# autonomousvision/transfuser

Hardware: AMD Instinct MI355X
Metric: training samples/sec (RGB+LiDAR pair), bs=10/GPU (higher is better)
Workload: dtype f32; 1 GPU; TransFuser LidarCenterNet (RegNetY-3.2GF x2, 168.0 M params) full train step, B=10/GPU, 3x256x704 RGB + 3x256x256 BEV, fp32, dropout 0.10, hipGraph replay; global_batch=10, parallelism=dp1, grad_allreduce=none (1 rank), build_id=e9ad36df01ded5b2

## Files before the change

### include/transfuser_hip.h

```cpp
#ifndef TRANSFUSER_HIP_H
#define TRANSFUSER_HIP_H
#include <stdint.h>
#ifdef __cplusplus
extern "C" {
#endif

int tf_version(void);
const char* tf_last_error(void);
const char* tf_build_id(void);
long tf_streamk_launches(void);

int tf_set_precision(int mode);
int tf_get_precision(void);
int tf_autotune(int enable);
int tf_force_plan(int bm, int bn, int bk, int splitk);
int tf_force_dma(int kind, int splitk);
int tf_plans_count(void);
int tf_plans_clear(void);
int tf_plans_save(const char* path);
int tf_plans_load(const char* path);


typedef struct {
    const float* a; const float* b; float* c; const float* bias; const float* res;
// ... 12 lines not shown
int tf_gemm_f32(const tf_gemm_desc* d, void* stream);
long tf_gemm_splitk_ws_floats(const tf_gemm_desc* d);
int tf_gemm_pair_begin(void);
int tf_gemm_pair_end(void* stream);
long tf_gemm_pair_count(int singles);

typedef struct {
    int B, Hi, Wi, Cin, Ho, Wo, Cout, ksize, stride, pad, groups;
} tf_conv_geom;
int tf_conv2d_fwd_f32(const tf_conv_geom* g, const float* x, const float* w, const float* bias, float* y, int relu, void* stream);
int tf_conv2d_fwd_colstat_f32(const tf_conv_geom* g, const float* x, const float* w, const float* bias, float* y, float* colstat, int* colstat_nparts,
                              void* stream);
int tf_conv2d_dgrad_f32(const tf_conv_geom* g, const float* dy, const float* w, float* dx, int accumulate, void* stream);
int tf_conv2d_wgrad_f32(const tf_conv_geom* g, const float* dy, const float* x, float* dw, int accumulate, void* stream);

int tf_conv3x3_small_fwd_f32(const float* x, const float* w, const float* bias, float* y, int B, int H, int W, int Cin, int Cout, int relu, void* stream);
int tf_conv3x3_small_dgrad_f32(const float* dy, const float* w, float* dx, int B, int H, int W, int Cin, int Cout, int accumulate, void* stream);
long tf_conv3x3_small_wgrad_ws_floats(void);
int tf_conv3x3_small_wgrad_f32(const float* dy, const float* x, float* dw, int B, int H, int W, int Cin, int Cout, int accumulate, float* ws, void* stream);

int tf_bn_finalize_parts_f32(const float* parts, int nparts, int rows, int C, const float* gamma, const float* beta, float* running_mean, float* running_var,
                             float momentum, float eps, float* save_mean, float* save_invstd, float* coef_out, void* stream);
int tf_colsum_bnrelu_parts_f32(const float* x, const float* coef, int nseg, int rows_per_seg, int C, float* ws, int* nchunks, void* stream);
int tf_se_excite_fwd_parts_f32(const float* parts, int nchunks, float scale, const float* W1, const float* b1, const float* W2, const float* b2, int B, int C,
                               int Cr, float* s_out, float* g1, float* gate, float* bwd_scratch, void* stream);
int tf_se_scale_bn_fwd_f32(const float* x, const float* coef, const float* gate, float* y, int B, int HW, int C, void* stream);
int tf_se_gate_grad_parts_f32(const float* dy, const float* x, const float* coef, int B, int HW, int C, float* ws, int* nchunks, void* stream);
int tf_se_excite_bwd_parts_f32(const float* parts, int nchunks, const float* gate, const float* s, const float* g1, const float* W1, const float* W2, int B,
                               int C, int Cr, float* dW1, float* db1, float* dW2, float* db2, float* ds, float* scratch, int scratch_is_zero, void* stream);
int tf_bn_bwd_remask_f32(const float* dz, const float* x, const float* fwd_coef, int rows, int C, const float* gamma, const float* save_mean,
                         const float* save_invstd, float* dx, float* dgamma, float* dbeta, float* ws, void* stream);
int tf_bn_bwd_remask_se_f32(const float* dy, const float* gate, const float* dmean, int B, int HW, int C, const float* x, const float* fcoef, const float* gamma,
                            const float* save_mean, const float* save_invstd, float* dx, float* dgamma, float* dbeta, float* ws, void* stream);

int tf_dwconv7_fwd_f32(const float* x, const float* w, const float* bias, float* y, int B, int H, int W, int C, int flip, int accumulate, void* stream);
int tf_dwconv7_wgrad_f32(const float* dy, const float* x, float* dw, float* dbias, int B, int H, int W, int C, void* stream);
int tf_gelu_fwd_f32(const float* x, float* y, int64_t n, void* stream);
int tf_gelu_bwd_f32(const float* dy, const float* x, float* dx, int64_t n, void* stream);
int tf_colscale_add_f32(const float* x, const float* gamma, const float* beta, const float* res, float* y, int64_t rows, int C, void* stream);
int tf_colsum_mul_f32(const float* a, const float* b, int rows, int C, float* out, int accumulate, float* ws, void* stream);
int tf_colsum_multi_f32(int n, const float* const* xs, const int* Cs, const long* lds, float* const* outs, int rows, void* stream);

int tf_cast16_f32(const float* x, int rows, int cols, int ldx, void* y16, int ldy, void* y16t, int ldyt, int dtype, void* stream);
typedef struct { const float* x; void* y16; void* y16t; int rows, cols, ldx, ldy, ldyt, tile0; } tf_cast16_item;
int tf_cast16_multi_f32(const tf_cast16_item* items_dev, int n_items, int total_tiles, int dtype, void* stream);
int tf_bn_apply16_f32(const float* x, const float* coef, const float* res, int relu, float* y32, int rows, int C, void* y16, void* y16t, int ldyt, int dtype, void* stream);
int tf_se_scale_bn16_f32(const float* x, const float* coef, const float* gate, int B, int HW, int C, void* y16, void* y16t, int ldyt, int dtype, void* stream);
int tf_bn_bwd16_f32(const float* dz, const float* z, const float* x, int rows, int C, const float* gamma, const float* save_mean, const float* save_invstd, float* dx32,
                    float* dres, float* dgamma, float* dbeta, float* ws, void* dx16, void* dx16t, int ldyt, int dtype, void* stream);
int tf_bn_bwd_remask16_f32(const float* dz, const float* x, const float* fcoef, int rows, int C, const float* gamma, const float* save_mean, const float* save_invstd,
                           float* dx32, float* dgamma, float* dbeta, float* ws, void* dx16, void* dx16t, int ldyt, int dtype, void* stream);
int tf_layernorm_fwd16_f32(const float* x, const float* gamma, const float* beta, void* y16, int ldy, void* y16t, int ldyt, float* mean, float* rstd,
                           int rows, int C, float eps, int dtype, void* stream);
int tf_gemm16_nt_f32(const void* a16, const void* b16, float* c, int m, int n, int k, int lda, int ldb, int ldc, const float* bias, const float* res, int ldres,
                     float alpha, int relu, int accumulate, const float* mask, int ldmask, int dtype, void* stream);
int tf_gemm16_nt_colstat_f32(const void* a16, const void* b16, float* c, int m, int n, int k, int lda, int ldb, int ldc, int dtype, float* colstat,
                             int* colstat_nparts, void* stream);
int tf_add_strided2_f32(const float* src, float* dst, int B, int Ho, int Wo, int C, int Hi, int Wi, void* stream);
int tf_im2col3x3_f32(const float* x, float* cols, int B, int H, int W, int C, void* stream);

int tf_conv3x3_thin_supported(int Cin, int Cout);
int tf_conv3x3_thin_fwd_f32(const float* x, const float* w, const float* bias, float* y, int B, int H, int W, int Cin, int Cout, void* stream);
int tf_conv3x3_thin_dgrad_f32(const float* dy, const float* w, const float* relu_mask, float* dx, int B, int H, int W, int Cin, int Cout, int accumulate,
                              void* stream);
long tf_conv3x3_thin_wgrad_ws_floats(void);
int tf_conv3x3_thin_wgrad_f32(const float* dy, const float* x, float* dw, float* dbias, int B, int H, int W, int Cin, int Cout, int accumulate, float* ws,
// ... 171 lines not shown
```

### transfuser_amd/csrc/reduce.cpp

```cpp
#include <cstdlib>
#include "tf_common.h"
#include "../../include/transfuser_hip.h"

using namespace tf;

namespace {

template <int V> struct vecf { float v[V]; };
template <int V> __device__ __forceinline__ vecf<V> ldv(const float* p) {
    vecf<V> r;
    if (V == 4) { float4 t = *reinterpret_cast<const float4*>(p); r.v[0] = t.x; r.v[1 % V] = t.y; r.v[2 % V] = t.z; r.v[3 % V] = t.w; }
    else r.v[0] = *p;
    return r;
}
template <int V> __device__ __forceinline__ void stv(float* p, const vecf<V>& a) {
    if (V == 4) *reinterpret_cast<float4*>(p) = make_float4(a.v[0], a.v[1 % V], a.v[2 % V], a.v[3 % V]);
    else *p = a.v[0];
}

constexpr int kBnSlots = 16;
constexpr int kMaxChunks = 512;
constexpr long kWsFloats = 4L << 20;
constexpr int kTickets = 4096;

// ... 593 lines not shown
    int e = 0;
#pragma unroll
    for (int i = 1; i < kMultiMax; ++i)
        if (i < d.n && (int)blockIdx.x >= d.strip0[i]) e = i;
    const int tx = threadIdx.x & 7, ty = threadIdx.x >> 3;
    const int C = d.C[e];
    const int c = ((int)blockIdx.x - d.strip0[e]) * 32 + tx * 4;
    const bool live = c < C;
    const float* p = d.x[e] + (live ? c : 0);
    const long ld = d.ld[e];
    float4 acc = make_float4(0.f, 0.f, 0.f, 0.f);
    int r = ty;
    for (; r + 7 * 32 < rows; r += 8 * 32) {
        float4 v[8];
#pragma unroll
        for (int u = 0; u < 8; ++u) v[u] = *reinterpret_cast<const float4*>(p + (long)(r + 32 * u) * ld);
#pragma unroll
        for (int u = 0; u < 8; ++u) { acc.x += v[u].x; acc.y += v[u].y; acc.z += v[u].z; acc.w += v[u].w; }
    }
    for (; r < rows; r += 32) {
        const float4 v = *reinterpret_cast<const float4*>(p + (long)r * ld);
        acc.x += v.x; acc.y += v.y; acc.z += v.z; acc.w += v.w;
    }
    red[ty][tx] = acc;
    __syncthreads();
    if (ty == 0 && live) {
        float4 t = make_float4(0.f, 0.f, 0.f, 0.f);
        for (int j = 0; j < 32; ++j) { const float4 v = red[j][tx]; t.x += v.x; t.y += v.y; t.z += v.z; t.w += v.w; }
        float* o = d.out[e] + c;
        o[0] += t.x; o[1] += t.y; o[2] += t.z; o[3] += t.w;
    }
}

constexpr int T16S = 64, T16P = T16S + 8;
template <class F>
__global__ void __launch_bounds__(256) tile16_kernel(F f, int rows, int C, uint16_t* __restrict__ y, uint16_t* __restrict__ yt, long ldyt, int f16) {
    __shared__ __attribute__((aligned(16))) uint16_t T[T16S * T16P];
    const int tid = threadIdx.x, r0 = blockIdx.y * T16S, c0 = blockIdx.x * T16S, c4 = (tid & 15) * 4;
#pragma unroll
    for (int it = 0; it < 4; ++it) {
        const int row = it * 16 + (tid >> 4), r = r0 + row, c = c0 + c4;
        float v[4] = {0.f, 0.f, 0.f, 0.f};
        const bool in = r < rows && c < C;
        if (in) f(r, c, v);
        uint16_t h[4];
#pragma unroll
        for (int e = 0; e < 4; ++e) h[e] = cvt16_bits(v[e], f16 != 0);
        if (y && in) *reinterpret_cast<float2*>(y + (long)r * C + c) = make_float2(__uint_as_float((uint32_t)h[0] | ((uint32_t)h[1] << 16)), __uint_as_float((uint32_t)h[2] | ((uint32_t)h[3] << 16)));
        if (yt) {
#pragma unroll
            for (int e = 0; e < 4; ++e) T[(c4 + e) * T16P + row] = h[e];
        }
    }
    if (!yt) return;
    __syncthreads();
    const int rows8 = (rows + 7) & ~7;
#pragma unroll
    for (int p = 0; p < 2; ++p) {
        const int id = p * 256 + tid, col = id >> 3, rc = (id & 7) * 8;
        if (c0 + col < C && r0 + rc < rows8) *reinterpret_cast<float4*>(yt + (long)(c0 + col) * ldyt + r0 + rc) = *reinterpret_cast<const float4*>(T + col * T16P + rc);
    }
}
struct BnApply16F {
    const float* x; const float* coef; const float* res; float* y32; int C; int relu;
    __device__ __forceinline__ void operator()(int r, int c, float (&v)[4]) const {
        const long o = (long)r * C + c;
// ... 229 lines not shown
    const bool v4 = (C % 4 == 0) && aligned16(dz) && aligned16(x) && aligned16(dx) && aligned16(fcoef);
    RedPlan p = plan_reduce(rows, C, 1, 2, v4);
    BnBwdRemaskF<4> f4{dz, x, fcoef, save_mean, save_invstd, C};
    BnBwdRemaskF<1> f1{dz, x, fcoef, save_mean, save_invstd, C};
    launch_reduce<2>(p, f4, f1, rows, C, 1, ws, stream);
    TF_LAUNCH(bn_bwd_finalize_kernel, dim3(cdiv(C, 4)), dim3(256), stream, (const float*)ws, gamma, save_mean, save_invstd, dgamma, dbeta, coef, C, p.nchunks,
              (float)rows);
    const long n = (long)rows * C;
    if (v4) TF_LAUNCH(bn_bwd_apply_remask_kernel<4>, dim3(ew_blocks(n / 4)), dim3(256), stream, dz, x, fcoef, (const float*)coef, dx, n / 4, C);
    else TF_LAUNCH(bn_bwd_apply_remask_kernel<1>, dim3(ew_blocks(n)), dim3(256), stream, dz, x, fcoef, (const float*)coef, dx, n, C);
    return launch_status("tf_bn_bwd_remask_f32");
}

extern "C" int tf_bn_bwd_remask_se_f32(const float* dy, const float* gate, const float* dmean, int B, int HW, int C, const float* x, const float* fcoef,
                                       const float* gamma, const float* save_mean, const float* save_invstd, float* dx, float* dgamma, float* dbeta, float* ws,
                                       void* stream) {
    TF_REQUIRE(dy && gate && dmean && x && fcoef && gamma && save_mean && save_invstd && dx && ws && B > 0 && HW > 0 && C > 0, "tf_bn_bwd_remask_se_f32: bad arguments");
    const int rows = B * HW;
    float* coef = ws + kWsFloats / 2;
    const bool v4 = (C % 4 == 0) && aligned16(dy) && aligned16(x) && aligned16(dx) && aligned16(fcoef) && aligned16(gate) && aligned16(dmean);
    RedPlan p = plan_reduce(rows, C, 1, 2, v4);
    const float inv_hw = 1.f / (float)HW;
    SeBnBwdRemaskF<4> f4{dy, gate, dmean, x, fcoef, save_mean, save_invstd, C, HW, inv_hw};
    SeBnBwdRemaskF<1> f1{dy, gate, dmean, x, fcoef, save_mean, save_invstd, C, HW, inv_hw};
    launch_reduce<2>(p, f4, f1, rows, C, 1, ws, stream);
    TF_LAUNCH(bn_bwd_finalize_kernel, dim3(cdiv(C, 4)), dim3(256), stream, (const float*)ws, gamma, save_mean, save_invstd, dgamma, dbeta, coef, C, p.nchunks,
              (float)rows);
    const long n = (long)rows * C;
    if (v4) TF_LAUNCH(bn_bwd_apply_remask_se_kernel<4>, dim3(ew_blocks(n / 4)), dim3(256), stream, dy, gate, dmean, x, fcoef, (const float*)coef, dx, n / 4, C, (long)HW * C / 4, inv_hw);
    else TF_LAUNCH(bn_bwd_apply_remask_se_kernel<1>, dim3(ew_blocks(n)), dim3(256), stream, dy, gate, dmean, x, fcoef, (const float*)coef, dx, n, C, (long)HW * C, inv_hw);
    return launch_status("tf_bn_bwd_remask_se_f32");
}

extern "C" int tf_colsum_mul_f32(const float* a, const float* b, int rows, int C, float* out, int accumulate, float* ws, void* stream) {
    TF_REQUIRE(a && b && out && ws && rows > 0 && C > 0, "tf_colsum_mul_f32: bad arguments");
    RedPlan p = plan_reduce(rows, C, 1, 1, aligned16(a) && aligned16(b));
    MulF<4> f4{a, b, C};
    MulF<1> f1{a, b, C};
    launch_reduce<1>(p, f4, f1, rows, C, 1, ws, stream);
    TF_LAUNCH(colsum_finalize_kernel, dim3(cdiv((long)C, 4)), dim3(256), stream, (const float*)ws, out, C, p.nchunks, 1, 1.f, accumulate);
    return launch_status("tf_colsum_mul_f32");
}

extern "C" int tf_colsum_multi_f32(int n, const float* const* xs, const int* Cs, const long* lds, float* const* outs, int rows, void* stream) {
    TF_REQUIRE(n >= 1 && n <= kMultiMax && xs && Cs && lds && outs && rows > 0, "tf_colsum_multi_f32: 1 <= n <= %d matrices with rows > 0", kMultiMax);
    MultiSum d;
    d.n = n;
    int strips = 0;
    for (int i = 0; i < kMultiMax; ++i) {
        const int j = i < n ? i : n - 1;
        d.x[i] = xs[j]; d.out[i] = outs[j]; d.C[i] = Cs[j]; d.ld[i] = lds[j];
        d.strip0[i] = strips;
        if (i < n) {
            TF_REQUIRE(xs[i] && outs[i] && Cs[i] > 0 && Cs[i] % 4 == 0 && lds[i] % 4 == 0 && lds[i] >= Cs[i] && aligned16(xs[i]),
                       "tf_colsum_multi_f32: entry %d needs C %% 4 == 0, ld %% 4 == 0, ld >= C and a 16-byte aligned base", i);
            strips += cdiv(Cs[i], 32);
        }
    }
    d.strip0[kMultiMax] = strips;
    TF_LAUNCH(colsum_multi_kernel, dim3(strips), dim3(256), stream, d, rows);
    return launch_status("tf_colsum_multi_f32");
}

extern "C" int tf_bn_apply16_f32(const float* x, const float* coef, const float* res, int relu, float* y32, int rows, int C, void* y16, void* y16t, int ldyt,
                                 int dtype, void* stream) {
    TF_REQUIRE(x && coef && tile16_ok(rows, C, y16, y16t, ldyt, dtype) && aligned16(x) && aligned16(coef) && (!res || aligned16(res)) && (!y32 || aligned16(y32)),
// ... 44 lines not shown
```

### transfuser_amd/functions.py

```python
import math

import torch

from . import ops


_INPLACE = False
_collect = None


class inplace_param_grads:
    def __enter__(self):
        global _INPLACE
        self.prev, _INPLACE = _INPLACE, True

    def __exit__(self, *a):
        global _INPLACE
        _INPLACE = self.prev


def gbuf(p):
    if _collect is not None:
        t = _collect.get(id(p))
        if t is None:
# ... 27 lines not shown
        finally:
            _collect = prev

    cls.forward, cls.backward = staticmethod(forward), staticmethod(backward)
    return cls


def w2d(w):
    return w.view(w.shape[0], w.shape[1])


def bias_grad(dy2d, b, mask2d=None):
    ops.colsum(dy2d, 1, dy2d.shape[0], dy2d.shape[1], 1.0, mask=mask2d, out=gbuf(b).view(1, -1), accumulate=True)


def _bn(x, bn, res=None, relu=False, stat=None):
    grp = getattr(bn, "_sync_group", None)
    if grp is None and isinstance(bn, torch.nn.SyncBatchNorm) and bn.training:
        import torch.distributed as dist
        if dist.is_available() and dist.is_initialized() and dist.get_world_size(bn.process_group) > 1:
            grp = bn.process_group if bn.process_group is not None else dist.group.WORLD
    if grp is not None and bn.training:
        return _bn_sync_fwd(x, bn, res, relu, grp)
    if stat is not None and bn.training:
        y, sm, si = ops.bn_fwd_parts(x, stat, bn.weight, bn.bias, bn.running_mean, bn.running_var, res, relu, bn.momentum, bn.eps)
        return y, (sm, si)
    y, sm, si = ops.bn_fwd(x, bn.weight, bn.bias, bn.running_mean, bn.running_var, res, relu, bn.training, bn.momentum, bn.eps)
    return y, (sm, si)


def _bn_bwd(dz, z, x, bn, st, want_dres=False):
    if len(st) == 4:
        return _bn_sync_bwd(dz, z, x, bn, st, want_dres)
    return ops.bn_bwd(dz, z, x, bn.weight, st[0], st[1], gbuf(bn.weight), gbuf(bn.bias), want_dres)


def convert_sync_batchnorm(model, group=None):
    import torch.distributed as dist
    grp = group if group is not None else dist.group.WORLD
    for m in model.modules():
        if isinstance(m, torch.nn.modules.batchnorm._BatchNorm):
            m._sync_group = grp
    return model


def _bn_sync_fwd(x, bn, res, relu, grp):
    import torch.distributed as dist
    C = x.shape[-1]
    n = x.numel() // C
    _, m_loc, i_loc = ops.bn_fwd(x, bn.weight, bn.bias, None, None, None, False, True, bn.momentum, bn.eps)
    world = dist.get_world_size(grp)
    mine = torch.cat([m_loc.double(), (1.0 / (i_loc.double() * i_loc.double()) - bn.eps).clamp_(min=0.0), torch.full((1,), float(n), dtype=torch.float64, device=x.device)])
    allst = [torch.empty_like(mine) for _ in range(world)]
    dist.all_gather(allst, mine, group=grp)
    cnt = torch.stack([t[2 * C] for t in allst])
    means = torch.stack([t[:C] for t in allst]); varis = torch.stack([t[C:2 * C] for t in allst])
    N = cnt.sum()
    mean = (means * cnt[:, None]).sum(0) / N
    var = ((varis + (means - mean) ** 2) * cnt[:, None]).sum(0) / N
    mean32, var32 = mean.float(), var.float()
    y, _, _ = ops.bn_fwd(x, bn.weight, bn.bias, mean32, var32, res, relu, False, bn.momentum, bn.eps)
    if bn.running_mean is not None:
        with torch.no_grad():
            mom = bn.momentum
            Nf = float(N)
            bn.running_mean.mul_(1 - mom).add_(mean32, alpha=mom)
            bn.running_var.mul_(1 - mom).add_(var32 * (Nf / (Nf - 1)) if Nf > 1 else var32, alpha=mom)
# ... 299 lines not shown
        else:
            out, st3 = _bn(y3, bn3, res=sc, relu=True, stat=cs3)
        ctx.saved = (x, blk, y1, z1, st1, y2, z2, st2, s, g1, gate, z2ss, y3, st3, yd, std, out, x2s, (lp, x16t, z16t))
        return out

    @staticmethod
    def backward(ctx, dout):
        if ctx.saved is None:
            raise RuntimeError("YBlockFn: trying to backward through the graph a second time: the saved activations are freed by the first backward "
                               "(retain_graph is not supported by the block Functions)")
        x, blk, y1, z1, st1, y2, z2, st2, s, g1, gate, z2ss, y3, st3, yd, std, out, x2s, (lp, x16t, z16t) = ctx.saved
        B, H, W, Cin = x.shape
        _, Ho, Wo, C = out.shape
        x2 = x.view(-1, Cin)
        w3 = blk.conv3.conv.weight
        if lp:
            bn3 = blk.conv3.bn
            if len(st3) == 2:
                _, d16, d16t, dsc = ops.bn_bwd16(dout.contiguous(), out, y3, bn3.weight, st3[0], st3[1], gbuf(bn3.weight), gbuf(bn3.bias), want_dres=True)
            else:
                dy3, dsc = _bn_bwd(dout.contiguous(), out, y3, bn3, st3, want_dres=True)
                d16, d16t = ops.cast16(dy3.view(-1, C))
            dz2s = _c1x1_bwd16(d16, d16t, z16t, w2d(w3), w2d(gbuf(w3))).view(B, Ho, Wo, C)
        else:
            dy3, dsc = _bn_bwd(dout.contiguous(), out, y3, blk.conv3.bn, st3, want_dres=True)
            dy3_2 = dy3.view(-1, C)
            dz2s = _c1x1_bwd(dy3_2, z2ss, w2d(w3), w2d(gbuf(w3))).view(B, Ho, Wo, C)
        se = blk.se
        if z2 is None:
            ds = ops.se_gate_excite_bn_bwd(dz2s, y2, st2[2], gate, s, g1, se.fc1.weight, se.fc2.weight, gbuf(se.fc1.weight), gbuf(se.fc1.bias),
                                           gbuf(se.fc2.weight), gbuf(se.fc2.bias))
            bn2 = blk.conv2.bn
            if ops.FUSE_SE_BN_BWD:
                dy2 = ops.bn_bwd_remask_se(dz2s, gate, ds, y2, st2[2], bn2.weight, st2[0], st2[1], gbuf(bn2.weight), gbuf(bn2.bias))
            else:
                dz2 = ops.se_scale_bwd_x(dz2s, gate, ds, y2.shape)
                dy2 = ops.bn_bwd_remask(dz2, y2, st2[2], bn2.weight, st2[0], st2[1], gbuf(bn2.weight), gbuf(bn2.bias))
        else:
            dgate = ops.se_scale_bwd_gate(dz2s, z2, gate)
            if B <= 16 and C <= ops.SE_FUSED_MAX_C and B * g1.shape[1] <= 8192:
                ds = ops.se_excite_bwd(dgate, s, g1, se.fc1.weight, se.fc2.weight, gbuf(se.fc1.weight), gbuf(se.fc1.bias), gbuf(se.fc2.weight),
                                       gbuf(se.fc2.bias))
            else:
                ops.linear_wgrad(dgate, g1, w2d(gbuf(se.fc2.weight)))
                bias_grad(dgate, se.fc2.bias)
                dg1 = ops.linear_dgrad(dgate, w2d(se.fc2.weight))
                dg1 = ops.relu_mask(dg1, g1, out=dg1)
                ops.linear_wgrad(dg1, s, w2d(gbuf(se.fc1.weight)))
                bias_grad(dg1, se.fc1.bias)
                ds = ops.linear_dgrad(dg1, w2d(se.fc1.weight))
            dz2 = ops.se_scale_bwd_x(dz2s, gate, ds, z2.shape)
            dy2, _ = _bn_bwd(dz2, z2, y2, blk.conv2.bn, st2)
        w2 = blk.conv2.conv.weight
        if z1 is None:
            bn1 = blk.conv1.bn
            ops.grouped_bnrelu_wgrad(dy2, y1, st1[2], gbuf(w2), stride=blk.stride)
            dz1 = ops.conv_dgrad(dy2, w2, y1.shape, blk.stride, 1, blk.groups)
            if lp:
                _, e16, e16t = ops.bn_bwd_remask16(dz1, y1, st1[2], bn1.weight, st1[0], st1[1], gbuf(bn1.weight), gbuf(bn1.bias))
            else:
                dy1 = ops.bn_bwd_remask(dz1, y1, st1[2], bn1.weight, st1[0], st1[1], gbuf(bn1.weight), gbuf(bn1.bias))
        else:
            ops.conv_wgrad(dy2, z1, gbuf(w2), blk.stride, 1, blk.groups)
            dz1 = ops.conv_dgrad(dy2, w2, z1.shape, blk.stride, 1, blk.groups)
            dy1, _ = _bn_bwd(dz1, z1, y1, blk.conv1.bn, st1)
            if lp:
                e16, e16t = ops.cast16(dy1.view(-1, C))
        w1 = blk.conv1.conv.weight
        if lp:
            c1b = lambda res=None: _c1x1_bwd16(e16, e16t, x16t, w2d(w1), w2d(gbuf(w1)), res=res)
        else:
            dy1_2 = dy1.view(-1, C)
            c1b = lambda res=None: _c1x1_bwd(dy1_2, x2s, w2d(w1), w2d(gbuf(w1)), res=res)
        if blk.downsample is None:
            dx = c1b(dsc.view(-1, Cin))
        else:
            dx = c1b()
            dyd, _ = _bn_bwd(dsc, None, yd, blk.downsample.bn, std)
            wd = blk.downsample.conv.weight
            if blk.stride == 1:
                ops.linear_wgrad(dyd.view(-1, C), x2, w2d(gbuf(wd)))
                ops.linear_dgrad(dyd.view(-1, C), w2d(wd), out=dx, accumulate=True)
            else:
                ops.conv_wgrad(dyd, x, gbuf(wd), blk.stride, 0, 1)
                ops.conv_dgrad(dyd, wd, x.shape, blk.stride, 0, 1, out=dx.view(B, H, W, Cin), accumulate=True)
        ctx.saved = None
        return (dx.view(B, H, W, Cin), None) + (None,) * (len(ctx.needs_input_grad) - 2)


def _attn_fwd(qkv, B, T, C, nh, drop=None):
    hs = C // nh
    Tp = (T + 3) // 4 * 4
    att = torch.empty(B * nh, T, Tp, dtype=torch.float32, device=qkv.device)
    k, q, v = qkv[:, :C], qkv[:, C:2 * C], qkv[:, 2 * C:]
# ... 642 lines not shown
```

### transfuser_amd/ops.py

```python
import ctypes

import os
import sys

import torch

from . import _lib
from ._lib import ConvGeom, GemmDesc, c_p, check, ptr, stream_of

byref = ctypes.byref

_ws_cache = {}


def L():
    return _lib.load()


def workspace(device):
    key = (str(device), torch.cuda.current_stream(device).cuda_stream if getattr(device, "type", str(device)[:4]) == "cuda" else 0)
    ws = _ws_cache.get(key)
    if ws is None:
        L().tf_workspace_bytes.restype = ctypes.c_long
        ws = torch.zeros(L().tf_workspace_bytes() // 4, dtype=torch.float32, device=device)
# ... 19 lines not shown
        if self.on:
            self._e = _census_begin()
            self._n0 = gemm_pair_count() if self._e is not None else 0
            _pair_shapes.clear()
            check(L().tf_gemm_pair_begin(), "tf_gemm_pair_begin")
            _pair_open[0] = True
        return self

    def __exit__(self, et, ev, tb):
        if self.on:
            _pair_open[0] = False
            rc = L().tf_gemm_pair_end(stream_of(self.t))
            if et is None:
                check(rc, "tf_gemm_pair_end")
                if self._e is not None and _pair_shapes:
                    joint = gemm_pair_count() > self._n0
                    _census_end(self._e, "gemm pair wgrad+dgrad (one grid)" if joint else "gemm wgrad+dgrad (two launches)", _pair_shapes[-1][:4], sum(v[4] for v in _pair_shapes))
        return False


def gemm_pair_count(singles=False):
    L().tf_gemm_pair_count.restype = ctypes.c_long
    return L().tf_gemm_pair_count(int(singles))


def autotune(enable):
    check(L().tf_autotune(int(bool(enable))), "tf_autotune")


def set_precision(mode):
    m = {"fp32": 0, "f32": 0, 0: 0, "bf16": 1, 1: 1, "f32x3": 2, "fp32x3": 2, "bf16x3": 2, 2: 2, "fp16": 3, "f16": 3, "half": 3, 3: 3}[mode]
    check(L().tf_set_precision(m), "tf_set_precision")
    _lowp["dtype"] = {1: 1, 3: 2}.get(m, 0) if _STORE16 else 0
    _lowp["w"].clear()
    _lowp.pop("table", None)


def get_precision():
    return ("fp32", "bf16", "f32x3", "fp16")[L().tf_get_precision()]


_STORE16 = os.environ.get("TF_STORE16", "1") != "0"
_lowp = {"dtype": 0, "managed": False, "w": {}}


def lowp_storage():
    return _lowp["dtype"]


def _t16():
    return torch.bfloat16 if _lowp["dtype"] == 1 else torch.float16


def cast16(x, want=True, want_t=True, out=None, out_t=None):
    rows, cols = x.shape
    assert x.stride(1) == 1
    rows8 = (rows + 7) // 8 * 8
    y = out if out is not None else (torch.empty(rows, cols, dtype=_t16(), device=x.device) if want else None)
    yt = out_t if out_t is not None else (torch.empty(cols, rows8, dtype=_t16(), device=x.device) if want_t else None)
    vp = lambda t: ctypes.c_void_p(t.data_ptr()) if t is not None else ctypes.c_void_p(0)
    check(L().tf_cast16_f32(ptr(x), rows, cols, x.stride(0), vp(y), y.stride(0) if y is not None else 0, vp(yt), yt.stride(0) if yt is not None else 0,
                            _lowp["dtype"], stream_of(x)), "tf_cast16_f32")
    return y, yt


def gemm16_nt(a16, b16, out, bias=None, res=None, relu=False, accumulate=False, mask=None, alpha=1.0, k=None, kind=0):
# ... 868 lines not shown
    g1 = buf[0]
    g1._bwd_scratch = buf[1]
    gate = torch.empty(B, C, dtype=torch.float32, device=y.device)
    check(L().tf_se_excite_fwd_parts_f32(ptr(ws), nch.value, ctypes.c_float(1.0 / (H * W)), wptr(w1), ptr(b1), wptr(w2), ptr(b2), B, C, Cr, ptr(s), ptr(g1),
                                         ptr(gate), ptr(buf[1]), stream_of(y)), "tf_se_excite_fwd_parts_f32")
    return s, g1, gate


def se_scale_bn_fwd(y, coef, gate):
    B, H, W, C = y.shape
    out = torch.empty_like(y)
    check(L().tf_se_scale_bn_fwd_f32(ptr(_c(y)), ptr(coef), ptr(_c(gate)), ptr(out), B, H * W, C, stream_of(y)), "tf_se_scale_bn_fwd_f32")
    return out


def se_gate_excite_bn_bwd(dz2s, y, coef, gate, s, g1, w1, w2, dw1, db1, dw2, db2):
    B, H, W, C = y.shape
    Cr = w1.shape[0]
    nch = ctypes.c_int(0)
    ws = workspace(y.device)
    check(L().tf_se_gate_grad_parts_f32(ptr(_c(dz2s)), ptr(_c(y)), ptr(coef), B, H * W, C, ptr(ws), byref(nch), stream_of(y)), "tf_se_gate_grad_parts_f32")
    ds = torch.empty(B, C, dtype=torch.float32, device=y.device)
    scratch = getattr(g1, "_bwd_scratch", None)
    zeroed = scratch is not None
    if zeroed:
        g1._bwd_scratch = None
    else:
        scratch = torch.empty(B, Cr, dtype=torch.float32, device=y.device)
    check(L().tf_se_excite_bwd_parts_f32(ptr(ws), nch.value, ptr(_c(gate)), ptr(_c(s)), ptr(_c(g1)), wptr(w1), wptr(w2), B, C, Cr, wptr(dw1), ptr(db1), wptr(dw2),
                                         ptr(db2), ptr(ds), ptr(scratch), int(zeroed), stream_of(y)), "tf_se_excite_bwd_parts_f32")
    return ds


def bn_bwd_remask(dz, x, coef, gamma, sm, si, dgamma, dbeta):
    C = x.shape[-1]
    rows = x.numel() // C
    dx = torch.empty_like(x)
    check(L().tf_bn_bwd_remask_f32(ptr(_c(dz)), ptr(_c(x)), ptr(coef), rows, C, ptr(gamma), ptr(sm), ptr(si), ptr(dx), ptr(dgamma), ptr(dbeta),
                                   ptr(workspace(x.device)), stream_of(x)), "tf_bn_bwd_remask_f32")
    return dx


FUSE_SE_BN_BWD = os.environ.get("TF_FUSE_SE_BN_BWD", "1") != "0"


def bn_bwd_remask_se(dy, gate, dmean, x, coef, gamma, sm, si, dgamma, dbeta):
    B, H, W, C = x.shape
    dx = torch.empty_like(x)
    _h = _hbm_begin()
    check(L().tf_bn_bwd_remask_se_f32(ptr(_c(dy)), ptr(gate), ptr(_c(dmean)), B, H * W, C, ptr(_c(x)), ptr(coef), ptr(gamma), ptr(sm), ptr(si), ptr(dx), ptr(dgamma),
                                      ptr(dbeta), ptr(workspace(x.device)), stream_of(x)), "tf_bn_bwd_remask_se_f32")
    _hbm_end(_h, "batchnorm backward (reduce + finalize + apply)", 4 * x.numel() * 5)
    return dx


def bn_bwd(dz, z, x, gamma, sm, si, dgamma, dbeta, want_dres=False):
    C = x.shape[-1]
    rows = x.numel() // C
    dx = torch.empty_like(x)
    dres = torch.empty_like(x) if want_dres else None
    zacc = zero_scratch(32 * C, x.device) if not _DBG_LEGACY_BNB else None
    _h = _hbm_begin()
    check(L().tf_bn_bwd_f32(ptr(_c(dz)), ptr(z), ptr(_c(x)), rows, C, ptr(gamma), ptr(sm), ptr(si), ptr(dx), ptr(dres), ptr(dgamma), ptr(dbeta),
                            ptr(workspace(x.device)), ptr(zacc), stream_of(x)), "tf_bn_bwd_f32")
    _hbm_end(_h, "batchnorm backward (reduce + finalize + apply)", 4 * x.numel() * ((2 + (z is not None)) * 2 + 1 + (dres is not None)))
    return dx, dres


FUSE_DROPOUT = os.environ.get("TF_FUSE_DROPOUT", "1") != "0"
LN_FWD16 = os.environ.get("TF_LN_FWD16", "1") != "0"


COLSUM_MULTI = os.environ.get("TF_COLSUM_MULTI", "1") != "0"


def colsum_multi(pairs):
    rows = pairs[0][0].shape[0]
    ok = 1 <= len(pairs) <= 8 and all(x.dim() == 2 and x.shape[0] == rows and x.stride(1) == 1 and x.shape[1] % 4 == 0 and x.stride(0) % 4 == 0 and
                                      x.data_ptr() % 16 == 0 and o.is_contiguous() and o.numel() == x.shape[1] for x, o in pairs)
    if not ok:
        for x, o in pairs:
            colsum(x.contiguous(), 1, rows, x.shape[1], 1.0, out=o.view(1, -1), accumulate=True)
        return
    n = len(pairs)
    xs = (ctypes.c_void_p * n)(*[x.data_ptr() for x, _ in pairs])
    outs = (ctypes.c_void_p * n)(*[o.data_ptr() for _, o in pairs])
    Cs = (ctypes.c_int * n)(*[x.shape[1] for x, _ in pairs])
    lds = (ctypes.c_long * n)(*[x.stride(0) for x, _ in pairs])
    check(L().tf_colsum_multi_f32(n, xs, Cs, lds, outs, rows, stream_of(pairs[0][0])), "tf_colsum_multi_f32")


def colsum(x, nseg, rows_per_seg, C, scale=1.0, mask=None, out=None, accumulate=False, pooled=False):
    if out is None:
# ... 497 lines not shown
```

Before: 228.8 samples/s.

## Add column-tiled two-kernel batchnorm backward with chunked partial sums

Adds a column-tiled batchnorm backward path: one kernel reduces per-chunk partial sums of grad and grad*x into a workspace, and a second kernel sums those partials in shared memory and applies the dx update over row chunks. It is used for the remask and SE-remask backward calls, but only on fp32 and when a heuristic says the shapes fit (rows per chunk small). The aim is to fill more of the GPU on small or narrow BN layers and avoid the older reduce/finalize/apply sequence. The plain bn_bwd path is gated behind a legacy debug flag, so it mostly stays on the old kernel.

```diff
diff --git a/include/transfuser_hip.h b/include/transfuser_hip.h
--- a/include/transfuser_hip.h
+++ b/include/transfuser_hip.h
@@ -68,6 +68,15 @@
                          const float* save_invstd, float* dx, float* dgamma, float* dbeta, float* ws, void* stream);
 int tf_bn_bwd_remask_se_f32(const float* dy, const float* gate, const float* dmean, int B, int HW, int C, const float* x, const float* fcoef, const float* gamma,
                             const float* save_mean, const float* save_invstd, float* dx, float* dgamma, float* dbeta, float* ws, void* stream);
+int tf_bn_bwd_cols_ok(int rows, int C);
+int tf_bn_bwd_cols_wins(int rows, int C);
+int tf_bn_bwd_cols_f32(const float* dz, const float* z, const float* x, int rows, int C, const float* gamma, const float* save_mean, const float* save_invstd,
+                       float* dx, float* dres, float* dgamma, float* dbeta, float* ws, void* stream);
+int tf_bn_bwd_remask_cols_f32(const float* dz, const float* x, const float* fwd_coef, int rows, int C, const float* gamma, const float* save_mean,
+                              const float* save_invstd, float* dx, float* dgamma, float* dbeta, float* ws, void* stream);
+int tf_bn_bwd_remask_se_cols_f32(const float* dy, const float* gate, const float* dmean, int B, int HW, int C, const float* x, const float* fcoef,
+                                 const float* gamma, const float* save_mean, const float* save_invstd, float* dx, float* dgamma, float* dbeta, float* ws,
+                                 void* stream);
 
 int tf_dwconv7_fwd_f32(const float* x, const float* w, const float* bias, float* y, int B, int H, int W, int C, int flip, int accumulate, void* stream);
 int tf_dwconv7_wgrad_f32(const float* dy, const float* x, float* dw, float* dbias, int B, int H, int W, int C, void* stream);
diff --git a/transfuser_amd/csrc/reduce.cpp b/transfuser_amd/csrc/reduce.cpp
--- a/transfuser_amd/csrc/reduce.cpp
+++ b/transfuser_amd/csrc/reduce.cpp
@@ -649,6 +649,199 @@
     }
 }
 
+constexpr int kBwdMaxChunks = 32;
+constexpr int kBwdCTV = 8, kBwdRL = 32, kBwdCols = kBwdCTV * 4;
+
+struct BwdPlan { int coltiles, nchunks, rows_per_chunk, achunks, arows_per_chunk; };
+inline BwdPlan plan_bn_bwd_cols(int rows, int C) {
+    BwdPlan p;
+    p.coltiles = cdiv(C, kBwdCols);
+    int want = cdiv(rows, kBwdRL * 4);
+    if (want > kBwdMaxChunks) want = kBwdMaxChunks;
+    const int blocks = p.coltiles * want;
+    if (blocks > 256) {
+        const int w2 = (blocks / 256) * 256 / p.coltiles;
+        if (w2 >= 1 && 2 * w2 > want) want = w2;
+    }
+    p.rows_per_chunk = cdiv(rows, want);
+    p.nchunks = cdiv(rows, p.rows_per_chunk);
+    int ac = cdiv(rows, kBwdRL * 8);
+    const int fill = cdiv(768, p.coltiles);
+    if (ac < fill) ac = fill;
+    const int acmax = cdiv(rows, kBwdRL * 4);
+    if (ac > acmax) ac = acmax;
+    p.arows_per_chunk = cdiv(rows, ac);
+    p.achunks = cdiv(rows, p.arows_per_chunk);
+    return p;
+}
+
+template <int UNR, class F>
+__global__ void __launch_bounds__(256) bn_bwd_reduce_parts_kernel(F f, int rows, int C, int rows_per_chunk, float* __restrict__ ws) {
+    __shared__ __attribute__((aligned(16))) float red[2][kBwdRL][kBwdCTV][4];
+    const int tid = threadIdx.x, cq = tid % kBwdCTV, rl = tid / kBwdCTV;
+    const int c0 = (blockIdx.x * kBwdCTV + cq) * 4;
+    const bool live = c0 < C;
+    const int c = live ? c0 : 0;
+    const int chunk = blockIdx.y;
+    const int r0 = chunk * rows_per_chunk;
+    int r1 = r0 + rows_per_chunk;
+    if (r1 > rows) r1 = rows;
+    vecf<4> acc[2];
+#pragma unroll
+    for (int a = 0; a < 2; ++a)
+#pragma unroll
+        for (int i = 0; i < 4; ++i) acc[a].v[i] = 0.f;
+    for (int r = r0 + rl; r < r1; r += UNR * kBwdRL) {
+        vecf<4> o[UNR][2];
+#pragma unroll
+        for (int u = 0; u < UNR; ++u) {
+            const int rr = r + u * kBwdRL;
+            f.eval(rr < r1 ? rr : r1 - 1, c, o[u]);
+        }
+#pragma unroll
+        for (int u = 0; u < UNR; ++u) {
+            const bool in = r + u * kBwdRL < r1;
+#pragma unroll
+            for (int a = 0; a < 2; ++a)
+#pragma unroll
+                for (int i = 0; i < 4; ++i) acc[a].v[i] += in ? o[u][a].v[i] : 0.f;
+        }
+    }
+#pragma unroll
+    for (int a = 0; a < 2; ++a)
+#pragma unroll
+        for (int i = 0; i < 4; ++i) red[a][rl][cq][i] = acc[a].v[i];
+    __syncthreads();
+    if (tid < 2 * kBwdCTV) {
+        const int a = tid / kBwdCTV, q = tid % kBwdCTV;
+        const int cw = (blockIdx.x * kBwdCTV + q) * 4;
+        vecf<4> t;
+#pragma unroll
+        for (int i = 0; i < 4; ++i) t.v[i] = 0.f;
+        for (int j = 0; j < kBwdRL; ++j)
+#pragma unroll
+            for (int i = 0; i < 4; ++i) t.v[i] += red[a][j][q][i];
+        if (cw < C) stv<4>(ws + ((long)chunk * 2 + a) * C + cw, t);
+    }
+}
+
+struct BwdGradZ {
+    const float* dz; const float* z; int C;
+    __device__ __forceinline__ vecf<4> grad(int row, int c, const vecf<4>&) const {
+        const long o = (long)row * C + c;
+        vecf<4> g = ldv<4>(dz + o);
+        if (z) { const vecf<4> zz = ldv<4>(z + o);
+#pragma unroll
+            for (int k = 0; k < 4; ++k) if (!(zz.v[k] > 0.f)) g.v[k] = 0.f; }
+        return g;
+    }
+};
+struct BwdGradRemask {
+    const float* dz; const float* fcoef; int C;
+    __device__ __forceinline__ vecf<4> grad(int row, int c, const vecf<4>& a) const {
+        vecf<4> g = ldv<4>(dz + (long)row * C + c);
+        const vecf<4> sc = ldv<4>(fcoef + c), sh = ldv<4>(fcoef + C + c);
+#pragma unroll
+        for (int k = 0; k < 4; ++k) if (!(a.v[k] * sc.v[k] + sh.v[k] > 0.f)) g.v[k] = 0.f;
+        return g;
+    }
+};
+struct BwdGradRemaskSe {
+    const float* dy; const float* gate; const float* dmean; const float* fcoef; int C; int HW; float inv_hw;
+    __device__ __forceinline__ vecf<4> grad(int row, int c, const vecf<4>& a) const {
+        const long bc = (long)(row / HW) * C + c;
+        vecf<4> g = ldv<4>(dy + (long)row * C + c);
+        const vecf<4> sc = ldv<4>(fcoef + c), sh = ldv<4>(fcoef + C + c), gt = ldv<4>(gate + bc), dm = ldv<4>(dmean + bc);
+#pragma unroll
+        for (int k = 0; k < 4; ++k) {
+            float gi = g.v[k] * (1.f / (1.f + expf(-gt.v[k]))) + dm.v[k] * inv_hw;
+            if (!(a.v[k] * sc.v[k] + sh.v[k] > 0.f)) gi = 0.f;
+            g.v[k] = gi;
+        }
+        return g;
+    }
+};
+
+template <class G>
+__global__ void __launch_bounds__(256) bn_bwd_apply_parts_kernel(G gf, const float* __restrict__ x, const float* __restrict__ ws, int nch,
+                                                                 const float* __restrict__ gamma, const float* __restrict__ mean,
+                                                                 const float* __restrict__ invstd, float* __restrict__ dgamma, float* __restrict__ dbeta,
+                                                                 float* __restrict__ dx, float* __restrict__ dres, int rows, int C, int rows_per_chunk,
+                                                                 float n) {
+    __shared__ float4 part[kBwdMaxChunks][2][kBwdCTV];
+    __shared__ float sum[2][kBwdCols];
+    const int tid = threadIdx.x, cq = tid % kBwdCTV, rl = tid / kBwdCTV;
+    const int tile0 = blockIdx.x * kBwdCols;
+    const int c0 = tile0 + cq * 4;
+    const bool live = c0 < C;
+    const int c = live ? c0 : 0;
+    float4 pv[2];
+#pragma unroll
+    for (int u = 0; u < 2; ++u) {
+        const int idx = tid + 256 * u, j = idx / (2 * kBwdCTV), a = (idx / kBwdCTV) % 2, q = idx % kBwdCTV;
+        const int cc = tile0 + q * 4;
+        pv[u] = (j < nch && cc < C) ? *reinterpret_cast<const float4*>(ws + ((long)j * 2 + a) * C + cc) : make_float4(0.f, 0.f, 0.f, 0.f);
+    }
+    const vecf<4> gm = ldv<4>(gamma + c), mu = ldv<4>(mean + c), is = ldv<4>(invstd + c);
+#pragma unroll
+    for (int u = 0; u < 2; ++u) {
+        const int idx = tid + 256 * u;
+        part[idx / (2 * kBwdCTV)][(idx / kBwdCTV) % 2][idx % kBwdCTV] = pv[u];
+    }
+    __syncthreads();
+    if (tid < 2 * kBwdCols) {
+        const int a = tid / kBwdCols, ch = tid % kBwdCols;
+        float s = 0.f;
+        for (int j = 0; j < nch; ++j) s += reinterpret_cast<const float*>(&part[j][a][0])[ch];
+        sum[a][ch] = s;
+    }
+    __syncthreads();
+    vecf<4> A, Bc, Cc;
+#pragma unroll
+    for (int i = 0; i < 4; ++i) {
+        const float sg = sum[0][cq * 4 + i], sgx = sum[1][cq * 4 + i];
+        if (blockIdx.y == 0 && rl == 0 && live) {
+            if (dgamma) dgamma[c + i] += sgx;
+            if (dbeta) dbeta[c + i] += sg;
+        }
+        A.v[i] = gm.v[i] * is.v[i];
+        Bc.v[i] = -A.v[i] * is.v[i] * (sgx / n);
+        Cc.v[i] = -A.v[i] * (sg / n) - Bc.v[i] * mu.v[i];
+    }
+    const int r0 = blockIdx.y * rows_per_chunk;
+    int r1 = r0 + rows_per_chunk;
+    if (r1 > rows) r1 = rows;
+    if (!live) return;
+    for (int r = r0 + rl; r < r1; r += 4 * kBwdRL) {
+        vecf<4> g[4], a[4];
+#pragma unroll
+        for (int u = 0; u < 4; ++u) {
+            const int rr = r + u * kBwdRL < r1 ? r + u * kBwdRL : r1 - 1;
+            a[u] = ldv<4>(x + (long)rr * C + c);
+            g[u] = gf.grad(rr, c, a[u]);
+        }
+#pragma unroll
+        for (int u = 0; u < 4; ++u) {
+            if (r + u * kBwdRL < r1) {
+                const long o = (long)(r + u * kBwdRL) * C + c;
+                if (dres) stv<4>(dres + o, g[u]);
+#pragma unroll
+                for (int k = 0; k < 4; ++k) a[u].v[k] = A.v[k] * g[u].v[k] + Bc.v[k] * a[u].v[k] + Cc.v[k];
+                stv<4>(dx + o, a[u]);
+            }
+        }
+    }
+}
+
+template <int UNR, class F, class G>
+inline void launch_bn_bwd_cols(const F& f, const G& g, const float* x, int rows, int C, const float* gamma, const float* mean, const float* invstd,
+                               float* dgamma, float* dbeta, float* dx, float* dres, float* ws, void* stream) {
+    const BwdPlan p = plan_bn_bwd_cols(rows, C);
+    TF_LAUNCH((bn_bwd_reduce_parts_kernel<UNR, F>), dim3(p.coltiles, p.nchunks), dim3(256), stream, f, rows, C, p.rows_per_chunk, ws);
+    TF_LAUNCH(bn_bwd_apply_parts_kernel<G>, dim3(p.coltiles, p.achunks), dim3(256), stream, g, x, (const float*)ws, p.nchunks, gamma, mean, invstd, dgamma,
+              dbeta, dx, dres, rows, C, p.arows_per_chunk, (float)rows);
+}
+
 constexpr int T16S = 64, T16P = T16S + 8;
 template <class F>
 __global__ void __launch_bounds__(256) tile16_kernel(F f, int rows, int C, uint16_t* __restrict__ y, uint16_t* __restrict__ yt, long ldyt, int f16) {
@@ -944,6 +1137,44 @@
     return launch_status("tf_bn_bwd_remask_se_f32");
 }
 
+extern "C" int tf_bn_bwd_cols_ok(int rows, int C) { return rows > 0 && C > 0 && C % 4 == 0 && (long)kBwdMaxChunks * 2 * C <= kWsFloats; }
+extern "C" int tf_bn_bwd_cols_wins(int rows, int C) {
+    if (!tf_bn_bwd_cols_ok(rows, C)) return 0;
+    const BwdPlan p = plan_bn_bwd_cols(rows, C);
+    return p.rows_per_chunk <= 8 * kBwdRL;
+}
+extern "C" int tf_bn_bwd_cols_f32(const float* dz, const float* z, const float* x, int rows, int C, const float* gamma, const float* save_mean,
+                                  const float* save_invstd, float* dx, float* dres, float* dgamma, float* dbeta, float* ws, void* stream) {
+    TF_REQUIRE(dz && x && gamma && save_mean && save_invstd && dx && ws && tf_bn_bwd_cols_ok(rows, C) && aligned16(dz) && aligned16(x) && aligned16(dx) &&
+               (!z || aligned16(z)) && (!dres || aligned16(dres)) && aligned16(gamma) && aligned16(save_mean) && aligned16(save_invstd) && aligned16(ws),
+               "tf_bn_bwd_cols_f32: needs C %% 4 == 0 and 16-byte aligned tensors");
+    launch_bn_bwd_cols<8>(BnBwdF<4>{dz, z, x, save_mean, save_invstd, C}, BwdGradZ{dz, z, C}, x, rows, C, gamma, save_mean, save_invstd, dgamma, dbeta, dx, dres,
+                          ws, stream);
+    return launch_status("tf_bn_bwd_cols_f32");
+}
+extern "C" int tf_bn_bwd_remask_cols_f32(const float* dz, const float* x, const float* fcoef, int rows, int C, const float* gamma, const float* save_mean,
+                                         const float* save_invstd, float* dx, float* dgamma, float* dbeta, float* ws, void* stream) {
+    TF_REQUIRE(dz && x && fcoef && gamma && save_mean && save_invstd && dx && ws && tf_bn_bwd_cols_ok(rows, C) && aligned16(dz) && aligned16(x) && aligned16(dx) &&
+               aligned16(fcoef) && aligned16(gamma) && aligned16(save_mean) && aligned16(save_invstd) && aligned16(ws),
+               "tf_bn_bwd_remask_cols_f32: needs C %% 4 == 0 and 16-byte aligned tensors");
+    launch_bn_bwd_cols<8>(BnBwdRemaskF<4>{dz, x, fcoef, save_mean, save_invstd, C}, BwdGradRemask{dz, fcoef, C}, x, rows, C, gamma, save_mean, save_invstd, dgamma,
+                          dbeta, dx, nullptr, ws, stream);
+    return launch_status("tf_bn_bwd_remask_cols_f32");
+}
+extern "C" int tf_bn_bwd_remask_se_cols_f32(const float* dy, const float* gate, const float* dmean, int B, int HW, int C, const float* x, const float* fcoef,
+                                            const float* gamma, const float* save_mean, const float* save_invstd, float* dx, float* dgamma, float* dbeta,
+                                            float* ws, void* stream) {
+    TF_REQUIRE(dy && gate && dmean && x && fcoef && gamma && save_mean && save_invstd && dx && ws && B > 0 && HW > 0 && (long)B * HW < (1L << 31) &&
+               tf_bn_bwd_cols_ok(B * HW, C) && aligned16(dy) && aligned16(x) && aligned16(dx) && aligned16(fcoef) && aligned16(gate) && aligned16(dmean) &&
+               aligned16(gamma) && aligned16(save_mean) && aligned16(save_invstd) && aligned16(ws),
+               "tf_bn_bwd_remask_se_cols_f32: needs C %% 4 == 0 and 16-byte aligned tensors");
+    const int rows = B * HW;
+    const float inv_hw = 1.f / (float)HW;
+    launch_bn_bwd_cols<4>(SeBnBwdRemaskF<4>{dy, gate, dmean, x, fcoef, save_mean, save_invstd, C, HW, inv_hw}, BwdGradRemaskSe{dy, gate, dmean, fcoef, C, HW, inv_hw},
+                          x, rows, C, gamma, save_mean, save_invstd, dgamma, dbeta, dx, nullptr, ws, stream);
+    return launch_status("tf_bn_bwd_remask_se_cols_f32");
+}
+
 extern "C" int tf_colsum_mul_f32(const float* a, const float* b, int rows, int C, float* out, int accumulate, float* ws, void* stream) {
     TF_REQUIRE(a && b && out && ws && rows > 0 && C > 0, "tf_colsum_mul_f32: bad arguments");
     RedPlan p = plan_reduce(rows, C, 1, 1, aligned16(a) && aligned16(b));
diff --git a/transfuser_amd/functions.py b/transfuser_amd/functions.py
--- a/transfuser_amd/functions.py
+++ b/transfuser_amd/functions.py
@@ -83,7 +83,7 @@
 def _bn_bwd(dz, z, x, bn, st, want_dres=False):
     if len(st) == 4:
         return _bn_sync_bwd(dz, z, x, bn, st, want_dres)
-    return ops.bn_bwd(dz, z, x, bn.weight, st[0], st[1], gbuf(bn.weight), gbuf(bn.bias), want_dres)
+    return ops.bn_bwd(dz, z, x, bn.weight, st[0], st[1], gbuf(bn.weight), gbuf(bn.bias), want_dres, cols=True)
 
 
 def convert_sync_batchnorm(model, group=None):
@@ -449,10 +449,10 @@
                                            gbuf(se.fc2.weight), gbuf(se.fc2.bias))
             bn2 = blk.conv2.bn
             if ops.FUSE_SE_BN_BWD:
-                dy2 = ops.bn_bwd_remask_se(dz2s, gate, ds, y2, st2[2], bn2.weight, st2[0], st2[1], gbuf(bn2.weight), gbuf(bn2.bias))
+                dy2 = ops.bn_bwd_remask_se(dz2s, gate, ds, y2, st2[2], bn2.weight, st2[0], st2[1], gbuf(bn2.weight), gbuf(bn2.bias), cols=True)
             else:
                 dz2 = ops.se_scale_bwd_x(dz2s, gate, ds, y2.shape)
-                dy2 = ops.bn_bwd_remask(dz2, y2, st2[2], bn2.weight, st2[0], st2[1], gbuf(bn2.weight), gbuf(bn2.bias))
+                dy2 = ops.bn_bwd_remask(dz2, y2, st2[2], bn2.weight, st2[0], st2[1], gbuf(bn2.weight), gbuf(bn2.bias), cols=True)
         else:
             dgate = ops.se_scale_bwd_gate(dz2s, z2, gate)
             if B <= 16 and C <= ops.SE_FUSED_MAX_C and B * g1.shape[1] <= 8192:
@@ -476,7 +476,7 @@
             if lp:
                 _, e16, e16t = ops.bn_bwd_remask16(dz1, y1, st1[2], bn1.weight, st1[0], st1[1], gbuf(bn1.weight), gbuf(bn1.bias))
             else:
-                dy1 = ops.bn_bwd_remask(dz1, y1, st1[2], bn1.weight, st1[0], st1[1], gbuf(bn1.weight), gbuf(bn1.bias))
+                dy1 = ops.bn_bwd_remask(dz1, y1, st1[2], bn1.weight, st1[0], st1[1], gbuf(bn1.weight), gbuf(bn1.bias), cols=True)
         else:
             ops.conv_wgrad(dy2, z1, gbuf(w2), blk.stride, 1, blk.groups)
             dz1 = ops.conv_dgrad(dy2, w2, z1.shape, blk.stride, 1, blk.groups)
diff --git a/transfuser_amd/ops.py b/transfuser_amd/ops.py
--- a/transfuser_amd/ops.py
+++ b/transfuser_amd/ops.py
@@ -75,6 +75,7 @@
     m = {"fp32": 0, "f32": 0, 0: 0, "bf16": 1, 1: 1, "f32x3": 2, "fp32x3": 2, "bf16x3": 2, 2: 2, "fp16": 3, "f16": 3, "half": 3, 3: 3}[mode]
     check(L().tf_set_precision(m), "tf_set_precision")
     _lowp["dtype"] = {1: 1, 3: 2}.get(m, 0) if _STORE16 else 0
+    _lowp["mode16"] = m in (1, 3)
     _lowp["w"].clear()
     _lowp.pop("table", None)
 
@@ -1009,10 +1010,23 @@
     return ds
 
 
-def bn_bwd_remask(dz, x, coef, gamma, sm, si, dgamma, dbeta):
+def _bn_bwd_cols(cols, rows, C, *tensors):
+    if cols is True and _lowp.get("mode16"):
+        return False
+    if not cols or not all(t is None or t.data_ptr() % 16 == 0 for t in tensors):
+        return False
+    return bool(L().tf_bn_bwd_cols_ok(rows, C)) if cols == "force" else bool(L().tf_bn_bwd_cols_wins(rows, C))
+
+
+def bn_bwd_remask(dz, x, coef, gamma, sm, si, dgamma, dbeta, cols=False):
     C = x.shape[-1]
     rows = x.numel() // C
     dx = torch.empty_like(x)
+    dz, x = _c(dz), _c(x)
+    if _bn_bwd_cols(cols, rows, C, dz, x, dx, coef, gamma, sm, si):
+        check(L().tf_bn_bwd_remask_cols_f32(ptr(dz), ptr(x), ptr(coef), rows, C, ptr(gamma), ptr(sm), ptr(si), ptr(dx), ptr(dgamma), ptr(dbeta),
+                                            ptr(workspace(x.device)), stream_of(x)), "tf_bn_bwd_remask_cols_f32")
+        return dx
     check(L().tf_bn_bwd_remask_f32(ptr(_c(dz)), ptr(_c(x)), ptr(coef), rows, C, ptr(gamma), ptr(sm), ptr(si), ptr(dx), ptr(dgamma), ptr(dbeta),
                                    ptr(workspace(x.device)), stream_of(x)), "tf_bn_bwd_remask_f32")
     return dx
@@ -1021,9 +1035,16 @@
 FUSE_SE_BN_BWD = os.environ.get("TF_FUSE_SE_BN_BWD", "1") != "0"
 
 
-def bn_bwd_remask_se(dy, gate, dmean, x, coef, gamma, sm, si, dgamma, dbeta):
+def bn_bwd_remask_se(dy, gate, dmean, x, coef, gamma, sm, si, dgamma, dbeta, cols=False):
     B, H, W, C = x.shape
     dx = torch.empty_like(x)
+    dy, dmean, x = _c(dy), _c(dmean), _c(x)
+    if _bn_bwd_cols(cols, B * H * W, C, dy, gate, dmean, x, dx, coef, gamma, sm, si):
+        _h = _hbm_begin()
+        check(L().tf_bn_bwd_remask_se_cols_f32(ptr(dy), ptr(gate), ptr(dmean), B, H * W, C, ptr(x), ptr(coef), ptr(gamma), ptr(sm), ptr(si), ptr(dx),
+                                               ptr(dgamma), ptr(dbeta), ptr(workspace(x.device)), stream_of(x)), "tf_bn_bwd_remask_se_cols_f32")
+        _hbm_end(_h, "batchnorm backward (reduce + apply)", 4 * x.numel() * 5)
+        return dx
     _h = _hbm_begin()
     check(L().tf_bn_bwd_remask_se_f32(ptr(_c(dy)), ptr(gate), ptr(_c(dmean)), B, H * W, C, ptr(_c(x)), ptr(coef), ptr(gamma), ptr(sm), ptr(si), ptr(dx), ptr(dgamma),
                                       ptr(dbeta), ptr(workspace(x.device)), stream_of(x)), "tf_bn_bwd_remask_se_f32")
@@ -1031,11 +1052,18 @@
     return dx
 
 
-def bn_bwd(dz, z, x, gamma, sm, si, dgamma, dbeta, want_dres=False):
+def bn_bwd(dz, z, x, gamma, sm, si, dgamma, dbeta, want_dres=False, cols=False):
     C = x.shape[-1]
     rows = x.numel() // C
     dx = torch.empty_like(x)
     dres = torch.empty_like(x) if want_dres else None
+    dz, x = _c(dz), _c(x)
+    if _DBG_LEGACY_BNB and _bn_bwd_cols(cols, rows, C, dz, z, x, dx, dres, gamma, sm, si):
+        _h = _hbm_begin()
+        check(L().tf_bn_bwd_cols_f32(ptr(dz), ptr(z), ptr(x), rows, C, ptr(gamma), ptr(sm), ptr(si), ptr(dx), ptr(dres), ptr(dgamma), ptr(dbeta),
+                                     ptr(workspace(x.device)), stream_of(x)), "tf_bn_bwd_cols_f32")
+        _hbm_end(_h, "batchnorm backward (reduce + apply)", 4 * x.numel() * ((2 + (z is not None)) * 2 + 1 + (dres is not None)))
+        return dx, dres
     zacc = zero_scratch(32 * C, x.device) if not _DBG_LEGACY_BNB else None
     _h = _hbm_begin()
     check(L().tf_bn_bwd_f32(ptr(_c(dz)), ptr(z), ptr(_c(x)), rows, C, ptr(gamma), ptr(sm), ptr(si), ptr(dx), ptr(dres), ptr(dgamma), ptr(dbeta),
```

Result: no change. 229.4 samples/s (median of 6 runs) (+0.3%).
